# LIS-TU-Berlin/SVN-ICP

Hardware: AMD Instinct MI355X
Metric: scan-pair registrations/sec at N particles x M source pts, 1/2/4/8 GPU (higher is better)
Workload: dtype f64; 1 GPU; C3: 128 particles SVN-ICP, 131072-pt source vs 262144-pt target, K=100, I=20, max_dist=1.0, lr=1.0, SVNFullGrad=False, correspondence=fast, early stop off; synthetic 64-beam scans (seed 20250718); particles=128, target_points=262144, knn_count=100, parallelism=single GPU

## Files before the change

svn-icp_amd/csrc/api.hip:

```cpp
#include "../../include/svnicp_hip.h"

#include <cmath>
#include <algorithm>
#include <cstdio>
#include <cstdlib>
#include <cstring>
#include <string>
#include <vector>

#include "device_buffer.hpp"
#include "information_solve.hpp"
#include "kernels.hpp"
#include "stage_a_host.hpp"
#include "stage_b_host.hpp"

using namespace svnicp;
using namespace svnicp_host;

namespace {

struct CloudState {
  DevBuf<double> src, tgt;
  bool src_set = false, tgt_set = false;
};

struct SteinState {
  DevBuf<double> init_pose, R, t, Rtot, pose_out, eul, opt, uctl, work, stats;
  DevBuf<float> history;
  DevBuf<int> ctl;
  int hist_I = 0, hist_P = 0;
  PinnedBuf<double> h_init, h_stats;
  bool host_stats_valid = false;
  Event ev_init;
  bool init_in_flight = false;
  StepPlan step;
  DrivePlan drive;
  int single_done_it = -1;
  Event ev_fork, ev_join;
  bool median_pending = false;
  DevBuf<unsigned int> small_bar;
  bool small_launched = false;
  Event ev_chunk[3];
  PinnedBuf<int> h_flags;
  bool finish_seen = true;
  int finish_iter = 0;
};

struct Sharding {
  int p_lo = 0, p_hi = 0;
  bool set = false;
  int row_rank = 0, row_world = 1;
  int64_t B_total = 0;
  DevBuf<double> rank_sums;
};

struct MiniBatch {
  int batch = 0;
  uint64_t seed = 0, n = 0;
  bool explicit_tab = false;
  int tab_I = 0;
  std::vector<int32_t> tab_h;
  int64_t tab_checked_B = -1;
// ... 349 lines not shown
  if (!name || !value) return fail(c, SVNICP_ERR_INVALID, "svnicp_set_option: null argument");
  const std::string k(name), v(value);
  Tuning& t = c->tune;
  auto num = [&](int lo, int hi, int* out) { char* end = nullptr; const long x = strtol(v.c_str(), &end, 10);
                                             if (end == v.c_str() || *end || x < lo || x > hi) return false; *out = (int)x; return true; };
  bool ok = true;
  if (k == "knn") { if (v == "auto") t.knn = {}; else if (v == "v1") t.knn = {false, KnnKernel::Stream}; else if (v == "v2") t.knn = {false, KnnKernel::SeededScan};
                    else if (v == "brute") t.knn = {false, KnnKernel::Brute}; else if (v == "tiles") t.knn = {false, KnnKernel::Tiles}; else ok = false; }
  else if (k == "knn_prefilter") { if (v == "mfma") t.knn_prefilter_mfma = 1; else if (v == "valu") t.knn_prefilter_mfma = 0; else ok = false; }
  else if (k == "fallback_sliced_max") ok = num(-1, 1 << 20, &t.fallback_sliced_max);
  else if (k == "accum") { if (v == "f64") t.accum = 0; else if (v == "valu") t.accum = 1; else if (v == "split") t.accum = 3; else ok = false; }
  else if (k == "update") { if (v == "auto") t.update_fused = 0; else if (v == "fused") t.update_fused = 1; else ok = false; }
  else if (k == "fused_update_max_p") ok = num(1, 700, &t.fused_update_max_p);
  else if (k == "wgpcu") { int x = 0, y = 0; ok = sscanf(v.c_str(), "%d,%d", &x, &y) == 2 && x >= 0 && x <= 64 && y >= 0 && y <= 16; if (ok) { t.wgpcu_search = x; t.wgpcu_accum = y; } }
  else if (k == "tp") ok = num(0, 1 << 16, &t.tp);
  else if (k == "debug") ok = num(0, 1, &t.debug);
  else if (k == "scan_split") ok = num(0, 16, &t.scan_split);
  else if (k == "group_stride") ok = num(0, 1 << 30, &t.group_stride);
  else if (k == "accum_min_steps") ok = num(0, 1 << 20, &t.accum_min_steps);
  else if (k == "brute_qb") { ok = num(0, 6, &t.brute_qb); }
  else if (k == "single") { if (v == "fused") t.single_fused = 1; else if (v == "split") t.single_fused = 0; else ok = false; }
  else if (k == "chain") { if (v == "auto") { t.small_chain = 1; t.persistent = 0; } else if (v == "persistent") { t.small_chain = 1; t.persistent = 1; }
                           else if (v == "general") { t.small_chain = 0; t.persistent = 0; } else ok = false; }
  else if (k == "median") { if (v == "auto") t.median_inline = -1; else if (v == "stream") t.median_inline = 0; else if (v == "inline") t.median_inline = 1; else ok = false; }
  else if (k == "sort") { if (v == "joint") t.sort_joint = 1; else if (v == "separate") t.sort_joint = 0; else ok = false; }
  else if (k == "sort_kernel") { if (v == "radix") t.sort_merge = 0; else if (v == "merge") t.sort_merge = 1; else ok = false; }
  else if (k == "table") { if (v == "select") t.table_select = 1; else if (v == "gather") t.table_select = 0; else ok = false; }
  else if (k == "correspondence") { if (v == "fast") t.full_corr = 0; else if (v == "full") t.full_corr = 1; else ok = false; }
  else return fail(c, SVNICP_ERR_INVALID, "svnicp_set_option: unknown option '" + k + "'");
  if (!ok) return fail(c, SVNICP_ERR_INVALID, "svnicp_set_option: bad value '" + v + "' for option '" + k + "'");
  c->run.have_candidates = false;
  c->sa.held = TargetLayout::None;
  if (c->run.began) c->st.step = plan_step(registration_facts(c, c->pl.on), c->tune, c->sb.plan);
  return SVNICP_OK;
}

int svnicp_set_shard(svnicp_ctx* c, int p_lo, int p_hi) {
  CTX_CHECK(c);
  if (!c->run.particles_set || p_lo < 0 || p_hi > c->P || p_lo > p_hi)
    return fail(c, SVNICP_ERR_INVALID, "svnicp_set_shard: need 0 <= p_lo <= p_hi <= P after svnicp_set_particles");
  c->shard.p_lo = p_lo; c->shard.p_hi = p_hi; c->shard.set = true;
  return SVNICP_OK;
}

int svnicp_set_row_shard(svnicp_ctx* c, int row_rank, int row_world, int64_t total_source_points) {
  CTX_CHECK(c);
  if (!c->run.particles_set || row_world < 1 || row_rank < 0 || row_rank >= row_world || (row_world > 1 && total_source_points < 1))
// ... 53 lines not shown
  if (r.mb) {
    HIPCHK(c, c->mb.idx.ensure((size_t)r.Bt)); HIPCHK(c, c->mb.flag.ensure((size_t)B)); HIPCHK(c, c->mb.pos.ensure((size_t)B));
    HIPCHK(c, c->mb.bsum.ensure((size_t)minibatch_scan_blocks(B))); HIPCHK(c, c->mb.ctl.ensure(2));
    HIPCHK(c, c->mb.src_u.ensure((size_t)r.Bq * 3)); HIPCHK(c, c->mb.src.ensure((size_t)r.Bt * 3));
    HIPCHK(c, c->mb.cand.ensure((size_t)r.Bt * c->K));
  }
  if (const int rc = c->sb.begin(c, f, c->tune, r, shape, c->num_cus)) return rc;
  HIPCHK(c, c->st.history.ensure((size_t)(I > 0 ? I : 1) * 6 * P));
  c->st.hist_I = I; c->st.hist_P = P;
  if (c->prm.record_trace) {
    const size_t IP = (size_t)I * P;
    HIPCHK(c, c->tr.corr.ensure(IP * r.Bi));
    HIPCHK(c, hipMemsetAsync(c->tr.corr.p, 0xff, IP * r.Bi * 4, c->stream));
    const struct { DevBuf<double>& buf; size_t n; } dbl[] = {{c->tr.H, IP * 36}, {c->tr.b, IP * 6}, {c->tr.N, IP * 6}, {c->tr.phi, IP * 6}, {c->tr.h, (size_t)I + 1}};
    for (const auto& x : dbl) {
      HIPCHK(c, x.buf.ensure(x.n));
      HIPCHK(c, hipMemsetAsync(x.buf.p, 0, x.n * 8, c->stream));
    }
  }
  c->prof.pused = 0;
  c->st.single_done_it = -1;
  if (c->st.median_pending) HIPCHK(c, hipStreamWaitEvent(c->stream, c->st.ev_join, 0));
  c->st.median_pending = false;
  if (!c->st.finish_seen && c->prm.mode == SVNICP_MODE_SVGD && c->prm.check_early_stop) {
    int v[2] = {0, 0};
    HIPCHK(c, hipMemcpyAsync(v, c->st.ctl.p, sizeof v, hipMemcpyDeviceToHost, c->stream));
    HIPCHK(c, hipStreamSynchronize(c->stream));
    if (v[0]) c->st.finish_iter = v[1];
    c->st.finish_seen = true;
  }
  {
    BeginZero z{};
    auto add = [&](void* p, size_t bytes) { if (p && bytes) { z.ptr[z.n] = static_cast<unsigned int*>(p); z.dwords[z.n] = (unsigned int)(bytes / 4); ++z.n; } };
    add(c->st.uctl.p, update_uctl_doubles(P) * sizeof(double));
    add(c->st.history.p, (size_t)(I > 0 ? I : 1) * 6 * P * sizeof(float));
    add(c->sb.ambig.p, 2 * sizeof(int));
    if (c->sa.plan.kernel == KnnKernel::Brute) add(c->sa.fail_count.p, sizeof(int));
    HIPCHK(c, c->st.small_bar.ensure(8));
    add(c->st.small_bar.p, 8 * sizeof(unsigned int));
    if (c->prm.mode == SVNICP_MODE_SVGD) add(c->st.opt.p, (size_t)P * 18 * sizeof(double));
    const bool sa_words = c->sa.layout_pending;
    if (sa_words) {
      add(c->sa.bbox.p + 3, 3 * sizeof(unsigned long long)); add(c->sa.emax.p, sizeof(unsigned long long)); add(c->sa.fail_count.p, sizeof(int));
      z.ones = reinterpret_cast<unsigned int*>(c->sa.bbox.p); z.ones_dwords = 6;
    }
    z.ctl = c->st.ctl.p; z.iterations = I;
// ... 170 lines not shown
  c->st.median_pending = true;
  return SVNICP_OK;
}

int svnicp_iter_accumulate(svnicp_ctx* c, int it) {
  CTX_CHECK(c);
  if (!c->run.began || !c->run.have_candidates)
    return fail(c, SVNICP_ERR_INVALID, "svnicp_iter_accumulate: candidates not staged");
  if (it < 0 || it >= c->prm.iterations) return fail(c, SVNICP_ERR_INVALID, "svnicp_iter_accumulate: bad iteration");
  if (bind(c)) return SVNICP_ERR_HIP;
  if (const int rc = fork_median(c, it)) return rc;
  const int nshard = c->shard.p_hi - c->shard.p_lo;
  if (nshard <= 0) return SVNICP_OK;
  AccumArgs a = accum_args(c, it);
  if (c->tune.full_corr) {
    HIPCHK(c, prof_begin(c, KC_SEARCH));
    for (int p = c->shard.p_lo; p < c->shard.p_hi; ++p) {
      HIPCHK(c, launch_transform_cloud(c->cloud.src.p, c->B, c->st.Rtot.p + 12 * (size_t)p, c->sb.full_q.p, c->st.ctl.p, c->stream));
      if (const int rc = c->sa.search_blocks(c, stage_a_env(c), c->sb.full_q.p, c->B, 1, c->sb.full_idx.p + (size_t)p * c->B, c->sb.full_d2.p, 1)) return rc;
    }
    HIPCHK(c, prof_end(c));
    a.full_idx = c->sb.full_idx.p;
  } else if (c->sb.plan.f32 == 3) {
    HIPCHK(c, prof_begin(c, KC_SEARCH));
    HIPCHK(c, launch_search_split(c->sb.plan, a, c->stream));
    HIPCHK(c, prof_end(c));
  }
  if (c->pl.on) {
    PlaneArgs pa{};
    pa.src = c->cloud.src.p; pa.rec = c->pl.rec.p; pa.Rtot = c->st.Rtot.p; pa.B = c->B; pa.M = c->M; pa.p_lo = c->shard.p_lo; pa.p_hi = c->shard.p_hi;
    pa.max_dist = c->prm.max_dist; pa.delta = c->pl.delta; pa.partial = c->pl.partial.p; pa.ctl = c->st.ctl.p;
    pa.kidx = c->sb.kidx.p; pa.kbest = c->sb.kbest.p; pa.corr = a.corr;
    HIPCHK(c, prof_begin(c, KC_ACCUM));
    HIPCHK(c, launch_plane_accumulate(c->sb.plan, pa, c->stream));
    HIPCHK(c, prof_end(c));
    HIPCHK(c, prof_begin(c, KC_REDUCE));
    HIPCHK(c, launch_plane_finalize(c->pl.partial.p, c->sb.plan.grid_x, c->sb.plan.Ppad, c->shard.p_lo, nshard, c->pl.Hb.p, c->pl.stats.p,
                                    c->st.ctl.p, c->stream));
    HIPCHK(c, prof_end(c));
    return SVNICP_OK;
  }
  const bool single = c->st.step.single_fused;
  const UpdateArgs us = update_args(c, it);
  HIPCHK(c, prof_begin(c, KC_ACCUM));
  HIPCHK(c, launch_accumulate(c->sb.plan, a, single ? &us : nullptr, c->stream));
  HIPCHK(c, prof_end(c));
  if (single) { c->st.single_done_it = it; return SVNICP_OK; }
  if (c->st.step.chain == StepChain::SmallChain) return SVNICP_OK;
  HIPCHK(c, prof_begin(c, KC_REDUCE));
// ... 8 lines not shown
  if (!c->run.began) return fail(c, SVNICP_ERR_INVALID, "svnicp_iter_update: call svnicp_align_begin first");
  if (it < 0 || it >= c->prm.iterations) return fail(c, SVNICP_ERR_INVALID, "svnicp_iter_update: bad iteration");
  if (bind(c)) return SVNICP_ERR_HIP;
  if (c->st.single_done_it == it) { c->st.single_done_it = -1; return SVNICP_OK; }
  if (const int rc = ensure_dbg_upd(c)) return rc;
  UpdateArgs u = update_args(c, it);
  HIPCHK(c, prof_begin(c, KC_UPDATE));
  if (c->tune.debug && it == c->prm.iterations - 1)
    if (const int rc = print_update_phases(c, false)) return rc;
  const StepChain chain = c->st.step.chain;
  if (chain == StepChain::OneKernel) {
    u.svgd = 0;
    if (c->prm.mode == SVNICP_MODE_SVGD) HIPCHK(c, launch_update_svgd(u, c->stream));
    else HIPCHK(c, launch_update(u, c->stream));
  } else {
    if (chain == StepChain::SmallChain) {
      u.sums = c->sb.partial.p; u.n_ranks = c->sb.plan.grid_x; u.sums_stride = c->sb.plan.Ppad * kNSums; u.sums_out = c->sb.sums.p;
    }
    if (chain == StepChain::SideStream) {
      if (const int rc = fork_median(c, it)) return rc;
      HIPCHK(c, launch_update_prepare(u, c->stream));
      HIPCHK(c, hipStreamWaitEvent(c->stream, c->st.ev_join, 0));
      c->st.median_pending = false;
    } else {
      HIPCHK(c, launch_update_prepare_median(u, c->stream));
    }
    HIPCHK(c, launch_update_direction(u, c->stream, step_finishes(c, it)));
  }
  HIPCHK(c, prof_end(c));
  return SVNICP_OK;
}

static int enqueue_scoring(svnicp_ctx* c, double gate) {
  const bool normals = c->pl.supplied || c->pl.estimated;
  if (score_tile_rows(c->P, c->K, normals) < 1)
    return fail(c, SVNICP_ERR_INVALID, std::string(kScoringRefusal) + "knn_count is too large for one row's candidates to fit the scoring kernel's LDS tile");
  ScoreState& sc = c->sc;
  sc.have = false;
  HIPCHK(c, sc.partial.ensure((size_t)score_blocks(c->B) * score_padded_particles(c->P, c->K) * kScoreRecord));
  HIPCHK(c, sc.scores.ensure((size_t)c->P * kScoreFields));
  HIPCHK(c, sc.poses.ensure((size_t)c->P * 12));
  ScoreArgs a{};
  a.src = c->cloud.src.p; a.tgt = c->cloud.tgt.p; a.rec = normals ? c->pl.rec.p : nullptr; a.cand = c->sa.cand_idx.p; a.Rtot = c->st.Rtot.p;
  a.B = c->B; a.M = c->M; a.K = c->K; a.P = c->P; a.thr2 = gate * gate; a.partial = sc.partial.p;
  HIPCHK(c, launch_particle_score(a, sc.scores.p, c->stream));
  HIPCHK(c, hipMemcpyAsync(sc.poses.p, c->st.Rtot.p, (size_t)c->P * 12 * sizeof(double), hipMemcpyDeviceToDevice, c->stream));
// ... 656 lines not shown
```

svn-icp_amd/csrc/kernels.hpp:

```cpp
#pragma once
#include "device_math.hpp"
#include "registration_plan.hpp"
#include "stage_a_plan.hpp"

namespace svnicp {

struct KnnArgs {
  const double* src;
  Pose0 pose;
  const double *tx, *ty, *tz;
  const int32_t* torig;
  int64_t M, Mp;
  int64_t b_lo, b_hi;
  int K, S;
  double* pool_d;
  int32_t* pool_i;
  int32_t* out_idx;
  double* out_d2;
  const int32_t* qlist;
  const int* qlist_count;
  int list_grid;
  int list_qw;
  int slices, slice_max_queries, merge_n;
  double* sl_d;
// ... 106 lines not shown
  int tiles_per_block;
  int64_t n_tiles;
  int Ppad;
  double max_dist;
  double* partial;
  const int* ctl;
  int32_t* corr;
  int svgd;
  const double* tgt;
  const int32_t* cand;
  const double* anchor;
  int64_t M;
  uint8_t* kbest;
  int32_t* kidx;
  const int32_t* full_idx;
  int pts_per_block, spts_per_block;
  unsigned int* ticket;
  int fin_iteration, fin_P;
  double fin_thr;
  const double* fin_norms;
  const double* fin_pose;
  float* fin_history;
  int* fin_ctl;
};
AccumPlan plan_accumulate(AccumPlan shape, int64_t B, int num_cus, const Tuning& tune);
hipError_t launch_search_split(const AccumPlan& plan, AccumArgs a, hipStream_t st);
hipError_t launch_accumulate_split(const AccumPlan& plan, const AccumArgs& a, hipStream_t st);
void split_occupancy_blocks(int PW, int WP, int K, size_t smem, int* search, int* accum);
hipError_t launch_build_table3(const int32_t* idx, int64_t B, int K, const double* tgt, int64_t M, double* table,
                               double* anchor, float4* tablea, float* cmax, hipStream_t st);
hipError_t launch_build_table3_list(const int32_t* idx, const int32_t* list, const int* count, int64_t B, int K, const double* tgt,
                                    int64_t M, double* anchor, float4* tablea, float* cmax, hipStream_t st);
hipError_t launch_build_table2(const int32_t* idx, int64_t B, int K, const double* tgt, int64_t M, double* table,
                               float4* tablef, float* cmax, hipStream_t st);
hipError_t launch_transform_cloud(const double* src, int64_t B, const double* pose12, double* q, const int* ctl, hipStream_t st);
struct UpdateArgs {
  const double* sums;
  int n_ranks;
  int sums_stride;
  double* sums_out;
  double* R;
  double* t;
  double* Rtot;
  Pose0 pose;
  int P, iteration, iterations;
  double lr, conv_thr;
// ... 152 lines not shown
```

svn-icp_amd/csrc/registration_plan.hpp:

```cpp
#pragma once
#include <cstddef>
#include <cstdint>
#include <initializer_list>

#include "stage_a_plan.hpp"

namespace svnicp {

struct Tuning {
  KnnOption knn;
  int knn_prefilter_mfma = 1;
  int fallback_sliced_max = -1;
  int accum = 3;
  int update_fused = 0;
  int fused_update_max_p = 128;
  int wgpcu_search = 0, wgpcu_accum = 0;
  int tp = 0;
  int accum_min_steps = 0;
  int group_stride = 0;
  int scan_split = 0;
  int debug = 0;
  int single_fused = 1;
  int small_chain = 1;
  int persistent = 0;
// ... 142 lines not shown
  AccumPlan pl = stage_b_shape(stage_b_variant(t.accum, f.K, f.nshard(), t.full_corr != 0, f.plane), f.nshard(), f.K);
  pl.small = small_registration(pl, f, t, Bi) ? 1 : 0;
  return pl;
}

inline bool select_writes_table(const RegistrationFacts& f, const Tuning& t, const StageAPlan& a, const AccumPlan& b) {
  return t.table_select && a.kernel == KnnKernel::Tiles && a.K == f.K && b.f32 == 3 && f.batch == 0 && !f.shard_set;
}

inline bool joint_morton_sort(const RegistrationFacts& f, const Tuning& t, const StageAPlan& a) {
  return t.sort_joint && a.kernel == KnnKernel::Tiles && a.rows == f.B && f.batch == 0 && !f.shard_set;
}

enum class StepChain {
  OneKernel,
  SmallChain,
  InlineMedian,
  SideStream,
};
constexpr int kMedianInlineMaxP = 128;

struct StepPlan {
  StepChain chain = StepChain::OneKernel;
  bool single_fused = false;
};
inline StepPlan plan_step(const RegistrationFacts& f, const Tuning& t, const AccumPlan& pl) {
  StepPlan s;
  if (f.P < 2 || (t.update_fused && f.P <= t.fused_update_max_p)) s.chain = StepChain::OneKernel;
  else if (pl.small) s.chain = StepChain::SmallChain;
  else if (f.P <= kMedianInlineMaxP && f.P <= t.fused_update_max_p && t.median_inline != 0) s.chain = StepChain::InlineMedian;
  else s.chain = StepChain::SideStream;
  s.single_fused = f.P == 1 && !f.svgd && f.row_world == 1 && f.p_lo == 0 && f.p_hi == 1 && !t.full_corr && t.single_fused && pl.f32 == 1 &&
                   !f.plane;
  return s;
}

inline bool small_registration_supported(int PW, int WP, int K) {
  return K >= 97 && K <= 100 && ((WP == 1 && (PW == 16 || PW == 32 || PW == 64)) || (PW == 64 && WP == 2));
}

constexpr int kChunk = 4;
struct DrivePlan {
  bool persistent_try = false;
  bool defer_fin = false;
  bool follow = false;
};
inline DrivePlan plan_drive(const RegistrationFacts& f, const Tuning& t, const AccumPlan& pl, const StepPlan& s, bool blocking) {
  DrivePlan d;
  d.persistent_try = s.chain == StepChain::SmallChain && t.persistent && !f.record_trace && !f.profiling && f.I > 0 &&
                     small_registration_supported(pl.PW, pl.WP, f.K);
  d.defer_fin = f.check_early_stop && !f.record_trace && pl.f32 == 3 && !t.full_corr && s.chain != StepChain::OneKernel;
  d.follow = blocking && f.check_early_stop && f.I > 2 * kChunk;
  return d;
}
// ... 3 lines not shown
```

svn-icp_amd/csrc/stein_split.hip:

```cpp
#include "stein_split_device.hpp"

namespace svnicp {

namespace {

__device__ __forceinline__ void build_table3_row(const int32_t* __restrict__ idx, int64_t b, int K, const double* __restrict__ tgt, int64_t M,
                                                 double* __restrict__ table, double* __restrict__ anchor, float4* __restrict__ tablea,
                                                 float* __restrict__ cmax, float* rb, int lane) {
  int64_t i0 = idx[b * K];
  i0 = i0 < 0 ? 0 : (i0 >= M ? M - 1 : i0);
  const double a0 = tgt[3 * i0], a1 = tgt[3 * i0 + 1], a2 = tgt[3 * i0 + 2];
  float cm = 0.0f;
  for (int k = lane; k < 128; k += kWave) {
    float4 row = table_sentinel_row();
    if (k < K) {
      int64_t i = idx[b * K + k];
      i = i < 0 ? 0 : (i >= M ? M - 1 : i);
      const double x = tgt[3 * i], y = tgt[3 * i + 1], z = tgt[3 * i + 2];
      if (table) {
        double* o = table + ((size_t)b * K + k) * 3;
        o[0] = x; o[1] = y; o[2] = z;
      }
      row = table_row(x, y, z, a0, a1, a2);
      cm = table_row_cmax(cm, row);
// ... 21 lines not shown
}

constexpr int kTableListGrid = 64;
__global__ __launch_bounds__(256) void k_build_table3_list(const int32_t* __restrict__ idx, const int32_t* __restrict__ list,
                                                           const int* __restrict__ count, int64_t B, int K,
                                                           const double* __restrict__ tgt, int64_t M, double* __restrict__ anchor,
                                                           float4* __restrict__ tablea, float* __restrict__ cmax) {
  __shared__ __align__(16) float rowbuf[4][128 * 4];
  const int lane = threadIdx.x & (kWave - 1), wave = threadIdx.x >> 6;
  const int64_t n = *count;
  for (int64_t e = (int64_t)blockIdx.x * 4 + wave; e < n && e < B; e += (int64_t)gridDim.x * 4) {
    const int64_t b = list[e];
    if (b < 0 || b >= B) continue;
    build_table3_row(idx, b, K, tgt, M, nullptr, anchor, tablea, cmax, rowbuf[wave], lane);
    __builtin_amdgcn_wave_barrier();
  }
}


inline int row_code_for(int K) { return K <= 16 ? 1 : K <= 32 ? 2 : K <= 64 ? 4 : K <= 96 ? 6 : K <= 100 ? 60 : K <= 112 ? 7 : 8; }

template <int PW, int WP, int NRB, bool TAIL>
hipError_t launch_s(const AccumPlan& plan, const AccumArgs& a, hipStream_t st) {
  hipLaunchKernelGGL((k_stein_search_bf16<PW, WP, NRB, TAIL>), dim3(plan.sgrid_x, plan.grid_y), dim3(NT), 0, st, a);
  return hipGetLastError();
}
template <int PW, int WP>
hipError_t launch_srb(const AccumPlan& plan, const AccumArgs& a, hipStream_t st) {
  switch (row_code_for(a.K)) {
    case 1: return launch_s<PW, WP, 1, false>(plan, a, st);
    case 2: return launch_s<PW, WP, 2, false>(plan, a, st);
    case 4: return launch_s<PW, WP, 4, false>(plan, a, st);
    case 6: return launch_s<PW, WP, 6, false>(plan, a, st);
    case 60: return launch_s<PW, WP, 6, true>(plan, a, st);
    case 7: return launch_s<PW, WP, 7, false>(plan, a, st);
    default: return launch_s<PW, WP, 8, false>(plan, a, st);
  }
}
template <int PW, int WP>
hipError_t launch_w(const AccumPlan& plan, const AccumArgs& a, hipStream_t st) {
  if (!a.svgd && !a.corr && !a.full_idx) hipLaunchKernelGGL((k_stein_accumulate_w<PW, WP, true>), dim3(plan.grid_x, plan.grid_y), dim3(NT), plan.smem, st, a);
  else if (a.svgd && !a.corr && !a.full_idx) hipLaunchKernelGGL((k_stein_accumulate_w<PW, WP, true, true>), dim3(plan.grid_x, plan.grid_y), dim3(NT), plan.smem, st, a);
  else hipLaunchKernelGGL((k_stein_accumulate_w<PW, WP, false>), dim3(plan.grid_x, plan.grid_y), dim3(NT), plan.smem, st, a);
  return hipGetLastError();
}

template <int PW, int WP, int NRB, bool TAIL>
// ... 24 lines not shown
void split_occupancy_blocks(int PW, int WP, int K, size_t smem, int* search, int* accum) {
  return dispatch_lanes(PW, WP, [&](auto l) { return occ_split<l.PW, l.WP>(K, smem, search, accum); });
}

hipError_t launch_build_table3(const int32_t* idx, int64_t B, int K, const double* tgt, int64_t M, double* table,
                               double* anchor, float4* tablea, float* cmax, hipStream_t st) {
  if (B <= 0) return hipSuccess;
  hipLaunchKernelGGL(k_build_table3, dim3((unsigned)((B + 3) / 4)), dim3(256), 0, st, idx, B, K, tgt, M, table, anchor, tablea,
                     cmax);
  return hipGetLastError();
}

hipError_t launch_build_table3_list(const int32_t* idx, const int32_t* list, const int* count, int64_t B, int K, const double* tgt,
                                    int64_t M, double* anchor, float4* tablea, float* cmax, hipStream_t st) {
  if (B <= 0) return hipSuccess;
  hipLaunchKernelGGL(k_build_table3_list, dim3(kTableListGrid), dim3(256), 0, st, idx, list, count, B, K, tgt, M, anchor, tablea, cmax);
  return hipGetLastError();
}


hipError_t launch_search_split(const AccumPlan& plan, AccumArgs a, hipStream_t st) {
  a.Ppad = plan.Ppad; a.pts_per_block = plan.pts_per_block; a.spts_per_block = plan.spts_per_block;
  if (!search_offsets_fit(a.Ppad, a.K)) return hipErrorInvalidValue;
  return dispatch_lanes(plan.PW, plan.WP, [&](auto l) { return launch_srb<l.PW, l.WP>(plan, a, st); });
}

__global__ __launch_bounds__(256) void k_transform_cloud(const double* __restrict__ src, int64_t B, const double* __restrict__ pose12,
                                                         double* __restrict__ q, const int* __restrict__ ctl) {
  if (ctl[0]) return;
  const int64_t b = (int64_t)blockIdx.x * blockDim.x + threadIdx.x;
  if (b >= B) return;
  const double s0 = src[3 * b], s1 = src[3 * b + 1], s2 = src[3 * b + 2];
  q[3 * b] = (s0 * pose12[0] + s1 * pose12[1] + s2 * pose12[2]) + pose12[9];
  q[3 * b + 1] = (s0 * pose12[3] + s1 * pose12[4] + s2 * pose12[5]) + pose12[10];
  q[3 * b + 2] = (s0 * pose12[6] + s1 * pose12[7] + s2 * pose12[8]) + pose12[11];
}

hipError_t launch_transform_cloud(const double* src, int64_t B, const double* pose12, double* q, const int* ctl, hipStream_t st) {
  if (B <= 0) return hipSuccess;
  hipLaunchKernelGGL(k_transform_cloud, dim3((unsigned)((B + 255) / 256)), dim3(256), 0, st, src, B, pose12, q, ctl);
  return hipGetLastError();
}

hipError_t launch_accumulate_split(const AccumPlan& plan, const AccumArgs& a, hipStream_t st) {
  return dispatch_lanes(plan.PW, plan.WP, [&](auto l) { return launch_w<l.PW, l.WP>(plan, a, st); });
}
// ... 3 lines not shown
```

svn-icp_amd/csrc/stein_split_device.hpp:

```cpp
#pragma once
#include <cstdlib>
#include "kernels.hpp"
#include "stein_common.hpp"
#include "lane_fold_device.hpp"
#include "search_limits.hpp"

namespace svnicp {

namespace {

typedef float v4f __attribute__((ext_vector_type(4)));
#define SVNICP_CONST_AS __attribute__((address_space(4)))

__device__ __forceinline__ float pack_slot(float v, unsigned int mask, unsigned int bits) {
  return __uint_as_float((__float_as_uint(v) & ~mask) | bits);
}
__device__ __forceinline__ float imin_f(float a, float b) {
  const int x = (int)__float_as_uint(a), y = (int)__float_as_uint(b);
  return __uint_as_float((unsigned int)(x < y ? x : y));
}
__device__ __forceinline__ float imax_f(float a, float b) {
  const int x = (int)__float_as_uint(a), y = (int)__float_as_uint(b);
  return __uint_as_float((unsigned int)(x > y ? x : y));
}

constexpr float kSentinelCC = 1.0e30f;
__device__ __forceinline__ float4 table_row(double x, double y, double z, double a0, double a1, double a2) {
  const float cx = (float)(x - a0), cy = (float)(y - a1), cz = (float)(z - a2);
// ... 93 lines not shown
    const double d = (dx * dx + dy * dy) + dz * dz;
    if (k == 0) d_first = d;
    if (k < K && (d < bd || (d == bd && k < bk))) { bd = d; bk = k; }
  }
#pragma unroll
  for (int off = G / 2; off > 0; off >>= 1) {
    const double od = __shfl_xor(bd, off, kWave);
    const int ok = __shfl_xor(bk, off, kWave);
    if (od < bd || (od == bd && ok < bk)) { bd = od; bk = ok; }
  }
  const double d0 = __shfl(d_first, (threadIdx.x & (kWave - 1)) & ~(G - 1), kWave);
  return (d0 != d0 || bk == 0x7fffffff) ? 0 : bk;
}

#ifndef SVNICP_SEARCH_EPS_U
#define SVNICP_SEARCH_EPS_U 54
#endif
constexpr float kEpsBf16 = (float)SVNICP_SEARCH_EPS_U * 5.9604644775390625e-08f;

#ifndef SVNICP_SEARCH_WAVES
#define SVNICP_SEARCH_WAVES 4
#endif
template <int PW, int WP, int NRB, bool TAIL>
__device__ __forceinline__ void search_body(const AccumArgs& a, int bx, int by) {
  if (a.ctl[0]) return;
  if (a.fin_iteration >= 0 && bx == 0 && by == 0) {
    __shared__ double sh_fin[NT];
    __shared__ int sh_fin_stop;
    const int ftid = threadIdx.x, FP = a.fin_P;
    double fs = 0.0;
    for (int p = ftid; p < FP; p += NT) fs += a.fin_norms[p];
    sh_fin[ftid] = fs;
    __syncthreads();
    for (int off = NT / 2; off > 0; off >>= 1) {
      if (ftid < off) sh_fin[ftid] += sh_fin[ftid + off];
      __syncthreads();
    }
    if (ftid == 0) {
      const double m = sh_fin[0] / FP;
      const int stop = (float)m < (float)a.fin_thr;
      if (stop) { a.fin_ctl[0] = 1; a.fin_ctl[1] = a.fin_iteration + 1; }
      sh_fin_stop = stop;
    }
    __syncthreads();
    if (sh_fin_stop) return;
    for (int e = ftid; e < 6 * FP; e += NT) a.fin_history[(size_t)a.fin_iteration * 6 * FP + e] = (float)a.fin_pose[e];
  }
  constexpr int BW = kWave / PW;
  constexpr int CBP = PW / 16;
  constexpr int NPT = 4 / CBP;
  constexpr int ST = 4 * BW;
  constexpr bool PIPE = NPT == 1;
  constexpr int NTILE = 4 * NRB + (TAIL ? 1 : 0);
  constexpr int RS = 16 * (((4 * NTILE + 15) / 16) | 1);
  __shared__ float4 s_rows[4][NPT][4][RS / 4];
  __shared__ float4 s_scr4[4][64];
  __shared__ double s_pose[WP][12][64];
  __shared__ unsigned int s_queue[kQueueCap];
  __shared__ unsigned int s_qn, s_qsteps;
  const int tid = threadIdx.x;
  if (tid == 0) { s_qn = 0u; s_qsteps = 0u; }
#pragma unroll
  for (int i = 0; i < kQueueCap / NT; ++i) s_queue[tid + i * NT] = 0xffffffffu;
  const int lane = tid & (kWave - 1);
  const int wave = __builtin_amdgcn_readfirstlane(tid >> 6);
  const int pl = lane % PW, bs = lane / PW;
  const int mj = lane & 15, mk = lane >> 4;
  const int pbase = by * (WP * PW);
  for (int g = wave; g < WP; g += 4) {
    const int p = a.p_lo + pbase + g * PW + pl;
    const double* rp = a.Rtot + 12 * (size_t)(p < a.p_hi ? p : a.p_lo);
#pragma unroll
    for (int i = 0; i < 12; ++i) s_pose[g][i][lane] = rp[i];
  }
  const int K = a.K;
  const SVNICP_CONST_AS v4f* ctab = (const SVNICP_CONST_AS v4f*)a.tablea;
  float* const rows_w = reinterpret_cast<float*>(&s_rows[wave][0][mk][0]) + mj;
  const int64_t blk_lo = (int64_t)bx * a.spts_per_block;
  const int64_t blk_hi = (blk_lo + a.spts_per_block < a.B) ? blk_lo + a.spts_per_block : a.B;
  static_assert(BW <= kSearchPointsPerStep, "search_limits.hpp bounds the pair offsets for at most this many points per step");
  __syncthreads();
  const int64_t nfirst = blk_lo + wave * BW;
// ... 238 lines not shown

  if (pend_have) *(int32_t*)((char*)pend_row + pend_off4) = pend_idx;
  __syncthreads();
  {
    const unsigned int total = s_qn < (unsigned int)kQueueCap ? s_qn : (unsigned int)kQueueCap;
    constexpr int kExactLanes = 32;
    const int sub = lane & (kExactLanes - 1);
    for (unsigned int e = (unsigned int)(tid / kExactLanes); e < total; e += NT / kExactLanes) {
      const unsigned int ent = s_queue[e];
      if (ent == 0xffffffffu) continue;
      const int64_t be = blk_lo + (int64_t)(ent >> 8);
      const int pin = (int)(ent & 0xffu);
      const int ke = exact_nearest_of_k<kExactLanes>(a, s_pose[pin / PW], be, pin % PW, K, sub);
      if (sub == 0) {
        a.kbest[(size_t)be * a.Ppad + (pbase + pin)] = (uint8_t)ke;
        a.kidx[(size_t)be * a.Ppad + (pbase + pin)] = a.cand[(size_t)be * K + ke];
      }
    }
    if (tid == 0 && a.ambig_count && s_qsteps) { atomicAdd(a.ambig_count, (int)s_qsteps); atomicAdd(a.ambig_count + 1, (int)s_qn); }
  }
}

template <int PW, int WP, int NRB, bool TAIL>
__global__ __launch_bounds__(NT, (PW == 16 || WP == 4) ? 3 : SVNICP_SEARCH_WAVES) void k_stein_search_bf16(AccumArgs a) {
  search_body<PW, WP, NRB, TAIL>(a, xcd_block((int)blockIdx.x, (int)gridDim.x), (int)blockIdx.y);
}

template <int PW, int WP, bool PLAIN, bool SVGD = false>
__device__ __forceinline__ void accumulate_body(const AccumArgs& a, int bx, int by, double* lds) {
  if (a.ctl[0]) return;
#ifndef SVNICP_ACCUM_U
#define SVNICP_ACCUM_U 4
#endif
  constexpr int U = SVNICP_ACCUM_U;
  using Lanes = ParticleLanes<PW, WP>;
  constexpr int BW = Lanes::BW, STEP = Lanes::STEP;
  const Lanes L(by);
  const int wb = L.wb, bs = L.bs, pidx = L.pidx;
  const int p = a.p_lo + pidx;
  const bool pvalid = p < a.p_hi;

  double Rt[9], tt[3];
  load_pose(a.Rtot + 12 * (size_t)(pvalid ? p : a.p_lo), Rt, tt);
  double acc[kNSums];
#pragma unroll
  for (int i = 0; i < kNSums; ++i) acc[i] = 0.0;
  const int K = a.K;
  const int64_t blk_lo = (int64_t)bx * a.pts_per_block;
// ... 129 lines not shown
```

svn-icp_amd/csrc/stein_step_device.hpp:

```cpp
#pragma once
#include "kernels.hpp"

namespace svnicp {
namespace {

constexpr int UT = 512;
constexpr int KREG = 32;

struct PhaseStamp {
  unsigned long long* dbg;
  unsigned long long t;
  __device__ PhaseStamp(unsigned long long* d, bool mine) : dbg(mine ? d : nullptr), t(d ? __builtin_readcyclecounter() : 0ull) {}
  __device__ __forceinline__ void operator()(int i) {
    if (!dbg) return;
    const unsigned long long now = __builtin_readcyclecounter();
    dbg[i] += now - t;
    t = now;
  }
};

__device__ inline void finalize_Hb(const double* s, const double* Rc, double* H, double* b) {
  const double sw = s[0];
  const double a0 = s[1], a1 = s[2], a2 = s[3];
  const double xx = s[4], xy = s[5], xz = s[6], yy = s[7], yz = s[8], zz = s[9];
// ... 190 lines not shown
      unsigned int incl = tot;
#pragma unroll
      for (int off = 1; off < kWave; off <<= 1) {
        const unsigned int v = __shfl_up(incl, off, kWave);
        if (lane >= off) incl += v;
      }
      unsigned int cum = incl - tot;
      const unsigned int rank = S->rank;
#pragma unroll
      for (int i = 0; i < 4; ++i) {
        if (rank >= cum && rank < cum + c[i]) {
          S->prefix = (pre << 8) | (unsigned long long)(4 * lane + i);
          S->rank = rank - cum;
        }
        cum += c[i];
      }
    }
    __syncthreads();
  }
  return S->prefix;
}

template <int T>
__device__ __attribute__((noinline)) void rbf_bandwidth(const double* lx, int P, double* sq_global, SelShared* S, int tid, int lane, int wave) {
  const int n = P * P;
  const bool keys_in_regs = n <= KREG * T;
  const float invP = 1.0f / (float)P;
  unsigned long long key[KREG];
  if (keys_in_regs) {
#pragma unroll
    for (int i = 0; i < KREG; ++i) {
      const int e = i * T + tid;
      key[i] = ~0ull;
      if (e < n) {
        int r = (int)((float)e * invP);
        if (r * P > e) --r;
        if ((r + 1) * P <= e) ++r;
        const double s = pair_sq(lx, r, e - r * P);
        key[i] = (unsigned long long)__double_as_longlong(s);
        if (s != s) S->nan_flag = 1;
      }
    }
  } else {
    for (int e = tid; e < n; e += T) {
      const int r = e / P;
      const double s = pair_sq(lx, r, e - r * P);
      sq_global[e] = s;
      if (s != s) S->nan_flag = 1;
    }
    __syncthreads();
  }
  const int nk = (n - tid + T - 1) / T;
  block_select([&](auto count) {
    if (keys_in_regs) {
#pragma unroll
      for (int i = 0; i < KREG; ++i)
        if (i < nk) count(key[i]);
    } else {
      for (int e = tid; e < n; e += T) count((unsigned long long)__double_as_longlong(sq_global[e]));
    }
  }, 7, S, lane, wave);
  if (tid == 0) {
    const double med = S->nan_flag ? __builtin_nan("") : __longlong_as_double((long long)S->prefix);
    S->h = med / log((double)(P + 1));
  }
  __syncthreads();
}

constexpr int UCTL_H = 2, UCTL_HINV = 3, UCTL_NAN = 40, UCTL_BIN = 42, UCTL_RANK = 43, UCTL_CNT = 44,
              UCTL_NORM = 64;
constexpr int HB_OCT = 48, HB_NB = HB_OCT * 256, HB_EXP0 = 1023 - 40;
constexpr int SEL_LDS_KEYS = 16384;
constexpr int COLL_CHUNK = 4096;

__device__ __forceinline__ int key_bin(unsigned long long k) {
  const long long kb = (long long)(k >> 44) - ((long long)HB_EXP0 << 8);
  return kb < 0 ? 0 : (kb >= HB_NB ? HB_NB - 1 : (int)kb);
}
__device__ __forceinline__ unsigned int* upd_hist(double* uctl, int P) {
  return reinterpret_cast<unsigned int*>(uctl + UCTL_NORM + ((P + 7) & ~7));
}

__device__ void svgd_gradient(const UpdateArgs& a, int p, double* g6);
__device__ double svgd_step_one(const UpdateArgs& a, int p, const double* phi6, const double* xold6);

constexpr int PREP_T = 256, PREP_CH = 128, PREP_PW = 64;
struct PrepShared { double H[PREP_CH][37]; double Hmean[36]; };

__device__ __forceinline__ void prepare_body(const UpdateArgs& a, int bx) {
  if (a.ctl[0]) return;
  __shared__ PrepShared sh;
  const int tid = threadIdx.x, P = a.P;
  Work w(a.work, P);
  const int n_pw = (P + PREP_PW - 1) / PREP_PW;
  if (bx < n_pw) {
    const int p = bx * PREP_PW + tid;
    if (tid >= PREP_PW || p >= P) return;
    if (a.svgd) {
      double g6[6];
      svgd_gradient(a, p, g6);
// ... 10 lines not shown
    for (int i = 0; i < 6; ++i) { w.b[p * 6 + i] = b[i]; w.N[p * 6 + i] = N[i]; }
    return;
  }
  double hsum = 0.0;
  for (int c0 = 0; c0 < P; c0 += PREP_CH) {
    const int p = c0 + tid;
    if (tid < PREP_CH && p < P) {
      double H[36], b[6];
      particle_Hb(a, p, H, b);
#pragma unroll
      for (int i = 0; i < 36; ++i) sh.H[tid][i] = H[i];
    }
    __syncthreads();
    const int cnt = P - c0 < PREP_CH ? P - c0 : PREP_CH;
    if (tid < 36)
      for (int q = 0; q < cnt; ++q) hsum += sh.H[q][tid];
    __syncthreads();
  }
  if (tid < 36) sh.Hmean[tid] = hsum / P;
  __syncthreads();
  if (tid < 6) inverse_column(sh.Hmean, tid, a.uctl + UCTL_HINV);
}

template <int T, class Hit>
__device__ __forceinline__ void bin_of_rank(const unsigned int* hist, unsigned int rank, unsigned int* wave_tot, Hit hit) {
  constexpr int CH = HB_NB / T;
  const int tid = threadIdx.x, lane = tid & (kWave - 1), wave = tid >> 6;
  unsigned int c[CH], tot = 0;
#pragma unroll
  for (int i = 0; i < CH; ++i) { c[i] = hist[tid * CH + i]; tot += c[i]; }
  unsigned int incl = tot;
#pragma unroll
  for (int off = 1; off < kWave; off <<= 1) {
    const unsigned int v = __shfl_up(incl, off, kWave);
    if (lane >= off) incl += v;
  }
  if (lane == kWave - 1) wave_tot[wave] = incl;
  __syncthreads();
  unsigned int cum = incl - tot;
  for (int wv = 0; wv < wave; ++wv) cum += wave_tot[wv];
#pragma unroll
  for (int i = 0; i < CH; ++i) {
    if (rank >= cum && rank < cum + c[i]) hit(tid * CH + i, rank - cum);
    cum += c[i];
  }
}

constexpr int FRONT_BUF = 2048;
template <int T>
__device__ __forceinline__ void median_body(const UpdateArgs& a) {
  if (a.ctl[0]) return;
  extern __shared__ __align__(16) double dyn[];
  const int tid = threadIdx.x, lane = tid & (kWave - 1), wave = tid >> 6;
  const int P = a.P;
  Work w(a.work, P);
  double* lx = dyn;
  double* lbuf = dyn + 6 * P;
  unsigned int* lh = reinterpret_cast<unsigned int*>(lbuf + FRONT_BUF + 8);
  __shared__ SelShared sel;
  __shared__ unsigned int sh_scan[T / kWave];
  __shared__ unsigned int sh_cnt;
  __shared__ int sh_bin, sh_rank, sh_nan;

  PhaseStamp stamp(a.dbg, tid == 0);
  for (int e = tid; e < HB_NB; e += T) lh[e] = 0u;
  if (tid == 0) { sh_cnt = 0u; sh_nan = 0; sh_bin = 0; sh_rank = 0; }
  for (int p = tid; p < P; p += T) {
#pragma unroll
    for (int d = 0; d < 6; ++d) { const double v = a.pose_out[d * P + p]; lx[p * 6 + d] = v; w.x[p * 6 + d] = v; }
  }
  __syncthreads();
  stamp(0);

  const int n = P * P;
  bool nan = false;
  constexpr int KH = ((KREG + 1) / 2 + 1) * (512 / T);
  const int Pe = P + (P & 1), W = Pe - 1, npair = (Pe / 2) * W;
  const int di = T / W, dj = T - di * W;
  double keys[KH];
  const int bin0 = key_bin(0ull);
  if (tid == 0) atomicAdd(&lh[bin0], (unsigned int)P);
  for (int p = tid; p < P; p += T) { const double sq = pair_sq(lx, p, p); if (sq != sq) nan = true; }
  {
    int ra = tid / W, c = tid - ra * W;
#pragma unroll
    for (int k = 0; k < KH; ++k) {
      const int e = tid + k * T;
      keys[k] = -1.0;
      const int i = c >= ra ? ra : Pe - 1 - ra, j = c >= ra ? c + 1 : Pe - 1 - c;
      if (e < npair && j < P) {
        const double sq = pair_sq(lx, i, j);
        if (sq != sq) nan = true;
        keys[k] = sq;
        atomicAdd(&lh[key_bin((unsigned long long)__double_as_longlong(sq))], 2u);
      }
      c += dj; ra += di;
      if (c >= W) { c -= W; ++ra; }
    }
  }
  if (nan) sh_nan = 1;
  __syncthreads();
  stamp(1);
  bin_of_rank<T>(lh, (unsigned int)((n - 1) / 2), sh_scan, [&](int bin, unsigned int inside) { sh_bin = bin; sh_rank = (int)inside; });
  __syncthreads();
  stamp(2);
  const int bstar = sh_bin;
#pragma unroll
  for (int k = 0; k < KH; ++k) {
    if (keys[k] >= 0.0 && key_bin((unsigned long long)__double_as_longlong(keys[k])) == bstar) {
      const unsigned int pos = atomicAdd(&sh_cnt, 1u);
      if (pos < FRONT_BUF) lbuf[pos] = keys[k];
    }
  }
  __syncthreads();
  stamp(3);
  const int m = (int)sh_cnt;
  double med;
  if (m <= FRONT_BUF) {
    const int r = sh_rank;
    const bool zin = bstar == bin0;
    for (int e = m + tid; e < ((m + 7) & ~7); e += T) lbuf[e] = __builtin_nan("");
    __syncthreads();
    for (int e = tid; e < m; e += T) {
      const double v = lbuf[e];
      int lt = 0, eq = 0;
      for (int j0 = 0; j0 < m; j0 += 8) {
        double u[8];
#pragma unroll
        for (int t = 0; t < 8; ++t) u[t] = lbuf[j0 + t];
#pragma unroll
        for (int t = 0; t < 8; ++t) { lt += u[t] < v ? 1 : 0; eq += u[t] == v ? 1 : 0; }
      }
      const int LT = 2 * lt + ((zin && 0.0 < v) ? P : 0), EQ = 2 * eq + ((zin && v == 0.0) ? P : 0);
      if (LT <= r && r < LT + EQ) sel.h = v;
    }
    if (zin && tid == 0) {
      int eq0 = 0;
      for (int j = 0; j < m; ++j) eq0 += lbuf[j] == 0.0 ? 1 : 0;
      if (r < 2 * eq0 + P) sel.h = 0.0;
    }
    __syncthreads();
    med = sel.h;
  } else {
    sel_init(&sel, lower_median_rank(P), 0ull, tid);
    __syncthreads();
    rbf_bandwidth<T>(lx, P, w.sq, &sel, tid, lane, wave);
    med = sel.h * log((double)(P + 1));
    __syncthreads();
  }
  stamp(4);
  if (tid == 0) a.uctl[UCTL_H] = (sh_nan ? __builtin_nan("") : med) / log((double)(P + 1));
}

__device__ __forceinline__ double rbf_pair(const double* xi, const double* xj, double h, double* df) {
  double sq = 0.0;
#pragma unroll
  for (int d = 0; d < 6; ++d) { df[d] = xi[d] - xj[d]; sq += df[d] * df[d]; }
  return exp(-sq / h);
}


__device__ __forceinline__ void stein_direction_default(const double* x, const double* N, const double* Hinv, int P, double h,
                                                        const double* xi, bool act, int part, int tpp, double* phi) {
  double g[6] = {0, 0, 0, 0, 0, 0}, kn[6] = {0, 0, 0, 0, 0, 0}, ks = 0.0;
  if (act)
    for (int j = part; j < P; j += tpp) {
      double df[6];
      const double k = rbf_pair(xi, x + j * 6, h, df);
#pragma unroll
      for (int d = 0; d < 6; ++d) {
        g[d] += df[d] * k;
        kn[d] += k * (-N[j * 6 + d]);
      }
      ks += k;
// ... 245 lines not shown
    }
    a.eul[i] = v;
    e6[d] = v;
    const double df = v - xold6[d];
    n2 += df * df;
  }
  double Rm[9], Rt[9], tt[3];
  euler_to_R(e6[3], e6[4], e6[5], Rm);
  mat3_mul(a.pose.R0, Rm, Rt);
  mat3_vec(a.pose.R0, e6, tt);
#pragma unroll
  for (int i = 0; i < 9; ++i) { a.R[9 * p + i] = Rm[i]; a.Rtot[12 * p + i] = Rt[i]; }
#pragma unroll
  for (int i = 0; i < 3; ++i) { a.t[3 * p + i] = e6[i]; a.Rtot[12 * p + 9 + i] = a.pose.t0[i] + tt[i]; }
#pragma unroll
  for (int d = 0; d < 6; ++d) a.pose_out[d * P + p] = e6[d];
  return sqrt(n2);
}

__host__ __device__ inline int prepare_blocks(const UpdateArgs& a) {
  return (a.P + PREP_PW - 1) / PREP_PW + ((!a.svgd && !a.full_grad) ? 1 : 0);
}
__host__ __device__ inline int direction_blocks(int P) { return (P + 3) / 4; }
inline size_t median_lds_bytes(int P) {
  return (size_t)P * 6 * sizeof(double) + (size_t)(FRONT_BUF + 8) * sizeof(double) + (size_t)HB_NB * sizeof(unsigned int);
}

}
}
```

Before: 150.0 registrations/s.

## Compute RBF bandwidth median in an extra block of the search kernel

```diff
diff --git a/svn-icp_amd/csrc/api.hip b/svn-icp_amd/csrc/api.hip
--- a/svn-icp_amd/csrc/api.hip
+++ b/svn-icp_amd/csrc/api.hip
@@ -38,6 +38,7 @@
   int single_done_it = -1;
   Event ev_fork, ev_join;
   bool median_pending = false;
+  int stats_done_it = -1;
   DevBuf<unsigned int> small_bar;
   bool small_launched = false;
   Event ev_chunk[3];
@@ -433,7 +434,7 @@
   else if (k == "single") { if (v == "fused") t.single_fused = 1; else if (v == "split") t.single_fused = 0; else ok = false; }
   else if (k == "chain") { if (v == "auto") { t.small_chain = 1; t.persistent = 0; } else if (v == "persistent") { t.small_chain = 1; t.persistent = 1; }
                            else if (v == "general") { t.small_chain = 0; t.persistent = 0; } else ok = false; }
-  else if (k == "median") { if (v == "auto") t.median_inline = -1; else if (v == "stream") t.median_inline = 0; else if (v == "inline") t.median_inline = 1; else ok = false; }
+  else if (k == "median") { if (v == "auto") t.median_inline = -1; else if (v == "stream") t.median_inline = 0; else if (v == "inline") t.median_inline = 1; else if (v == "search") t.median_inline = 2; else ok = false; }
   else if (k == "sort") { if (v == "joint") t.sort_joint = 1; else if (v == "separate") t.sort_joint = 0; else ok = false; }
   else if (k == "sort_kernel") { if (v == "radix") t.sort_merge = 0; else if (v == "merge") t.sort_merge = 1; else ok = false; }
   else if (k == "table") { if (v == "select") t.table_select = 1; else if (v == "gather") t.table_select = 0; else ok = false; }
@@ -533,6 +534,7 @@
   c->st.single_done_it = -1;
   if (c->st.median_pending) HIPCHK(c, hipStreamWaitEvent(c->stream, c->st.ev_join, 0));
   c->st.median_pending = false;
+  c->st.stats_done_it = -1;
   if (!c->st.finish_seen && c->prm.mode == SVNICP_MODE_SVGD && c->prm.check_early_stop) {
     int v[2] = {0, 0};
     HIPCHK(c, hipMemcpyAsync(v, c->st.ctl.p, sizeof v, hipMemcpyDeviceToHost, c->stream));
@@ -749,9 +751,16 @@
     HIPCHK(c, prof_end(c));
     a.full_idx = c->sb.full_idx.p;
   } else if (c->sb.plan.f32 == 3) {
+    const bool stats = c->st.step.stats_in_search;
+    if (stats) {
+      if (const int rc = ensure_dbg_upd(c)) return rc;
+      const UpdateArgs u = update_args(c, it);
+      a.stat_P = u.P; a.stat_pose = u.pose_out; a.stat_work = u.work; a.stat_uctl = u.uctl; a.stat_dbg = u.dbg;
+    }
     HIPCHK(c, prof_begin(c, KC_SEARCH));
     HIPCHK(c, launch_search_split(c->sb.plan, a, c->stream));
     HIPCHK(c, prof_end(c));
+    if (stats) c->st.stats_done_it = it;
   }
   if (c->pl.on) {
     PlaneArgs pa{};
@@ -806,6 +815,9 @@
       HIPCHK(c, launch_update_prepare(u, c->stream));
       HIPCHK(c, hipStreamWaitEvent(c->stream, c->st.ev_join, 0));
       c->st.median_pending = false;
+    } else if (c->st.stats_done_it == it) {
+      HIPCHK(c, launch_update_prepare(u, c->stream));
+      c->st.stats_done_it = -1;
     } else {
       HIPCHK(c, launch_update_prepare_median(u, c->stream));
     }
diff --git a/svn-icp_amd/csrc/kernels.hpp b/svn-icp_amd/csrc/kernels.hpp
--- a/svn-icp_amd/csrc/kernels.hpp
+++ b/svn-icp_amd/csrc/kernels.hpp
@@ -152,6 +152,11 @@
   const double* fin_pose;
   float* fin_history;
   int* fin_ctl;
+  int stat_P;
+  double* stat_pose;
+  double* stat_work;
+  double* stat_uctl;
+  unsigned long long* stat_dbg;
 };
 AccumPlan plan_accumulate(AccumPlan shape, int64_t B, int num_cus, const Tuning& tune);
 hipError_t launch_search_split(const AccumPlan& plan, AccumArgs a, hipStream_t st);
diff --git a/svn-icp_amd/csrc/registration_plan.hpp b/svn-icp_amd/csrc/registration_plan.hpp
--- a/svn-icp_amd/csrc/registration_plan.hpp
+++ b/svn-icp_amd/csrc/registration_plan.hpp
@@ -188,6 +188,7 @@
 
 struct StepPlan {
   StepChain chain = StepChain::OneKernel;
+  bool stats_in_search = false;
   bool single_fused = false;
 };
 inline StepPlan plan_step(const RegistrationFacts& f, const Tuning& t, const AccumPlan& pl) {
@@ -196,6 +197,9 @@
   else if (pl.small) s.chain = StepChain::SmallChain;
   else if (f.P <= kMedianInlineMaxP && f.P <= t.fused_update_max_p && t.median_inline != 0) s.chain = StepChain::InlineMedian;
   else s.chain = StepChain::SideStream;
+  const bool ride_asked = t.median_inline == 2 || (t.median_inline < 0 && s.chain == StepChain::InlineMedian);
+  s.stats_in_search = (s.chain == StepChain::SmallChain || s.chain == StepChain::InlineMedian) && pl.f32 == 3 && !t.full_corr && ride_asked &&
+                      f.nshard() > 0;
   s.single_fused = f.P == 1 && !f.svgd && f.row_world == 1 && f.p_lo == 0 && f.p_hi == 1 && !t.full_corr && t.single_fused && pl.f32 == 1 &&
                    !f.plane;
   return s;
diff --git a/svn-icp_amd/csrc/stein_split.hip b/svn-icp_amd/csrc/stein_split.hip
--- a/svn-icp_amd/csrc/stein_split.hip
+++ b/svn-icp_amd/csrc/stein_split.hip
@@ -67,7 +67,7 @@
 
 template <int PW, int WP, int NRB, bool TAIL>
 hipError_t launch_s(const AccumPlan& plan, const AccumArgs& a, hipStream_t st) {
-  hipLaunchKernelGGL((k_stein_search_bf16<PW, WP, NRB, TAIL>), dim3(plan.sgrid_x, plan.grid_y), dim3(NT), 0, st, a);
+  hipLaunchKernelGGL((k_stein_search_bf16<PW, WP, NRB, TAIL>), dim3(plan.sgrid_x + (a.stat_P > 0 ? 1 : 0), plan.grid_y), dim3(NT), 0, st, a);
   return hipGetLastError();
 }
 template <int PW, int WP>
@@ -138,6 +138,7 @@
 hipError_t launch_search_split(const AccumPlan& plan, AccumArgs a, hipStream_t st) {
   a.Ppad = plan.Ppad; a.pts_per_block = plan.pts_per_block; a.spts_per_block = plan.spts_per_block;
   if (!search_offsets_fit(a.Ppad, a.K)) return hipErrorInvalidValue;
+  if (a.stat_P != 0 && (a.stat_P < 2 || a.stat_P > kStatMaxP)) return hipErrorInvalidValue;
   return dispatch_lanes(plan.PW, plan.WP, [&](auto l) { return launch_srb<l.PW, l.WP>(plan, a, st); });
 }
 
diff --git a/svn-icp_amd/csrc/stein_split_device.hpp b/svn-icp_amd/csrc/stein_split_device.hpp
--- a/svn-icp_amd/csrc/stein_split_device.hpp
+++ b/svn-icp_amd/csrc/stein_split_device.hpp
@@ -4,6 +4,7 @@
 #include "stein_common.hpp"
 #include "lane_fold_device.hpp"
 #include "search_limits.hpp"
+#include "stein_step_device.hpp"
 
 namespace svnicp {
 
@@ -143,7 +144,19 @@
 #define SVNICP_SEARCH_WAVES 4
 #endif
 template <int PW, int WP, int NRB, bool TAIL>
-__device__ __forceinline__ void search_body(const AccumArgs& a, int bx, int by) {
+struct SearchLds {
+  static constexpr int NPT = 4 / (PW / 16);
+  static constexpr int NTILE = 4 * NRB + (TAIL ? 1 : 0);
+  static constexpr int RS = 16 * (((4 * NTILE + 15) / 16) | 1);
+  float4 rows[4][NPT][4][RS / 4];
+  float4 scr4[4][64];
+  double pose[WP][12][64];
+  unsigned int queue[kQueueCap];
+  unsigned int qn, qsteps;
+};
+
+template <int PW, int WP, int NRB, bool TAIL>
+__device__ __forceinline__ void search_body(const AccumArgs& a, int bx, int by, SearchLds<PW, WP, NRB, TAIL>& lds) {
   if (a.ctl[0]) return;
   if (a.fin_iteration >= 0 && bx == 0 && by == 0) {
     __shared__ double sh_fin[NT];
@@ -174,11 +187,12 @@
   constexpr bool PIPE = NPT == 1;
   constexpr int NTILE = 4 * NRB + (TAIL ? 1 : 0);
   constexpr int RS = 16 * (((4 * NTILE + 15) / 16) | 1);
-  __shared__ float4 s_rows[4][NPT][4][RS / 4];
-  __shared__ float4 s_scr4[4][64];
-  __shared__ double s_pose[WP][12][64];
-  __shared__ unsigned int s_queue[kQueueCap];
-  __shared__ unsigned int s_qn, s_qsteps;
+  static_assert(NPT == SearchLds<PW, WP, NRB, TAIL>::NPT && RS == SearchLds<PW, WP, NRB, TAIL>::RS, "SearchLds states the same geometry");
+  float4 (&s_rows)[4][NPT][4][RS / 4] = lds.rows;
+  float4 (&s_scr4)[4][64] = lds.scr4;
+  double (&s_pose)[WP][12][64] = lds.pose;
+  unsigned int (&s_queue)[kQueueCap] = lds.queue;
+  unsigned int &s_qn = lds.qn, &s_qsteps = lds.qsteps;
   const int tid = threadIdx.x;
   if (tid == 0) { s_qn = 0u; s_qsteps = 0u; }
 #pragma unroll
@@ -463,8 +477,41 @@
 }
 
 template <int PW, int WP, int NRB, bool TAIL>
+__device__ __forceinline__ void search_body(const AccumArgs& a, int bx, int by) {
+  __shared__ SearchLds<PW, WP, NRB, TAIL> lds;
+  search_body<PW, WP, NRB, TAIL>(a, bx, by, lds);
+}
+
+constexpr int kStatBins = 64, kStatFront = 1024, kStatMaxP = 128;
+constexpr size_t kStatLdsBytes = median_lds_bytes(kStatMaxP, kStatBins, kStatFront);
+static_assert(kStatLdsBytes == 26688, "x 6 144 + front buffer 8 256 + histogram 12 288 bytes at 128 particles");
+
+template <int PW, int WP, int NRB, bool TAIL>
+union SearchLaunchLds {
+  SearchLds<PW, WP, NRB, TAIL> search;
+  double stat[kStatLdsBytes / sizeof(double)];
+};
+constexpr size_t kSearchLdsBeside = NT * sizeof(double) + sizeof(SelShared) + 64;
+
+__device__ __forceinline__ void pair_stats_ride(const AccumArgs& a, double* lds) {
+  UpdateArgs u{};
+  u.P = a.stat_P; u.pose_out = a.stat_pose; u.work = a.stat_work; u.uctl = a.stat_uctl; u.dbg = a.stat_dbg;
+  u.ctl = const_cast<int*>(a.ctl);
+  median_body<NT, kStatBins, kStatFront, false>(u, lds);
+}
+
+template <int PW, int WP, int NRB, bool TAIL>
 __global__ __launch_bounds__(NT, (PW == 16 || WP == 4) ? 3 : SVNICP_SEARCH_WAVES) void k_stein_search_bf16(AccumArgs a) {
-  search_body<PW, WP, NRB, TAIL>(a, xcd_block((int)blockIdx.x, (int)gridDim.x), (int)blockIdx.y);
+  constexpr int kPerCu = (PW == 16 || WP == 4) ? 3 : SVNICP_SEARCH_WAVES;
+  static_assert(kPerCu * (sizeof(SearchLaunchLds<PW, WP, NRB, TAIL>) + kSearchLdsBeside) <= 160 * 1024,
+                "the workgroups of a CU share 160 KB of LDS: the statistics' bytes alias the search arrays, they do not add to them");
+  __shared__ SearchLaunchLds<PW, WP, NRB, TAIL> lds;
+  const int ride = a.stat_P > 0 ? 1 : 0;
+  if (ride && blockIdx.x == 0) {
+    if (blockIdx.y == 0) pair_stats_ride(a, lds.stat);
+    return;
+  }
+  search_body<PW, WP, NRB, TAIL>(a, xcd_block((int)blockIdx.x - ride, (int)gridDim.x - ride), (int)blockIdx.y, lds.search);
 }
 
 template <int PW, int WP, bool PLAIN, bool SVGD = false>
diff --git a/svn-icp_amd/csrc/stein_step_device.hpp b/svn-icp_amd/csrc/stein_step_device.hpp
--- a/svn-icp_amd/csrc/stein_step_device.hpp
+++ b/svn-icp_amd/csrc/stein_step_device.hpp
@@ -236,7 +236,7 @@
 }
 
 template <int T>
-__device__ __attribute__((noinline)) void rbf_bandwidth(const double* lx, int P, double* sq_global, SelShared* S, int tid, int lane, int wave) {
+__device__ __forceinline__ void rbf_bandwidth_inline(const double* lx, int P, double* sq_global, SelShared* S, int tid, int lane, int wave) {
   const int n = P * P;
   const bool keys_in_regs = n <= KREG * T;
   const float invP = 1.0f / (float)P;
@@ -280,6 +280,10 @@
   }
   __syncthreads();
 }
+template <int T>
+__device__ __attribute__((noinline)) void rbf_bandwidth(const double* lx, int P, double* sq_global, SelShared* S, int tid, int lane, int wave) {
+  rbf_bandwidth_inline<T>(lx, P, sq_global, S, tid, lane, wave);
+}
 
 constexpr int UCTL_H = 2, UCTL_HINV = 3, UCTL_NAN = 40, UCTL_BIN = 42, UCTL_RANK = 43, UCTL_CNT = 44,
               UCTL_NORM = 64;
@@ -287,9 +291,14 @@
 constexpr int SEL_LDS_KEYS = 16384;
 constexpr int COLL_CHUNK = 4096;
 
+constexpr int hb_bins(int BPO) { return HB_OCT * BPO; }
+constexpr int hb_log2(int BPO) { return BPO <= 1 ? 0 : 1 + hb_log2(BPO / 2); }
+template <int BPO = 256>
 __device__ __forceinline__ int key_bin(unsigned long long k) {
-  const long long kb = (long long)(k >> 44) - ((long long)HB_EXP0 << 8);
-  return kb < 0 ? 0 : (kb >= HB_NB ? HB_NB - 1 : (int)kb);
+  constexpr int LG = hb_log2(BPO), NB = hb_bins(BPO);
+  static_assert((1 << LG) == BPO && LG <= 8, "bins per octave: a power of two, at most 256");
+  const long long kb = (long long)(k >> (52 - LG)) - ((long long)HB_EXP0 << LG);
+  return kb < 0 ? 0 : (kb >= NB ? NB - 1 : (int)kb);
 }
 __device__ __forceinline__ unsigned int* upd_hist(double* uctl, int P) {
   return reinterpret_cast<unsigned int*>(uctl + UCTL_NORM + ((P + 7) & ~7));
@@ -346,9 +355,10 @@
   if (tid < 6) inverse_column(sh.Hmean, tid, a.uctl + UCTL_HINV);
 }
 
-template <int T, class Hit>
+template <int T, int NB = HB_NB, class Hit>
 __device__ __forceinline__ void bin_of_rank(const unsigned int* hist, unsigned int rank, unsigned int* wave_tot, Hit hit) {
-  constexpr int CH = HB_NB / T;
+  static_assert(NB % T == 0, "a whole chunk of bins per thread");
+  constexpr int CH = NB / T;
   const int tid = threadIdx.x, lane = tid & (kWave - 1), wave = tid >> 6;
   unsigned int c[CH], tot = 0;
 #pragma unroll
@@ -371,10 +381,13 @@
 }
 
 constexpr int FRONT_BUF = 2048;
-template <int T>
-__device__ __forceinline__ void median_body(const UpdateArgs& a) {
+constexpr size_t median_lds_bytes(int P, int bpo = 256, int front = FRONT_BUF) {
+  return (size_t)P * 6 * sizeof(double) + (size_t)(front + 8) * sizeof(double) + (size_t)hb_bins(bpo) * sizeof(unsigned int);
+}
+template <int T, int BPO, int FB, bool CALL = true>
+__device__ __forceinline__ void median_body(const UpdateArgs& a, double* dyn) {
   if (a.ctl[0]) return;
-  extern __shared__ __align__(16) double dyn[];
+  constexpr int HB_NB = hb_bins(BPO), FRONT_BUF = FB;
   const int tid = threadIdx.x, lane = tid & (kWave - 1), wave = tid >> 6;
   const int P = a.P;
   Work w(a.work, P);
@@ -402,7 +415,7 @@
   const int Pe = P + (P & 1), W = Pe - 1, npair = (Pe / 2) * W;
   const int di = T / W, dj = T - di * W;
   double keys[KH];
-  const int bin0 = key_bin(0ull);
+  const int bin0 = key_bin<BPO>(0ull);
   if (tid == 0) atomicAdd(&lh[bin0], (unsigned int)P);
   for (int p = tid; p < P; p += T) { const double sq = pair_sq(lx, p, p); if (sq != sq) nan = true; }
   {
@@ -416,7 +429,7 @@
         const double sq = pair_sq(lx, i, j);
         if (sq != sq) nan = true;
         keys[k] = sq;
-        atomicAdd(&lh[key_bin((unsigned long long)__double_as_longlong(sq))], 2u);
+        atomicAdd(&lh[key_bin<BPO>((unsigned long long)__double_as_longlong(sq))], 2u);
       }
       c += dj; ra += di;
       if (c >= W) { c -= W; ++ra; }
@@ -425,13 +438,13 @@
   if (nan) sh_nan = 1;
   __syncthreads();
   stamp(1);
-  bin_of_rank<T>(lh, (unsigned int)((n - 1) / 2), sh_scan, [&](int bin, unsigned int inside) { sh_bin = bin; sh_rank = (int)inside; });
+  bin_of_rank<T, HB_NB>(lh, (unsigned int)((n - 1) / 2), sh_scan, [&](int bin, unsigned int inside) { sh_bin = bin; sh_rank = (int)inside; });
   __syncthreads();
   stamp(2);
   const int bstar = sh_bin;
 #pragma unroll
   for (int k = 0; k < KH; ++k) {
-    if (keys[k] >= 0.0 && key_bin((unsigned long long)__double_as_longlong(keys[k])) == bstar) {
+    if (keys[k] >= 0.0 && key_bin<BPO>((unsigned long long)__double_as_longlong(keys[k])) == bstar) {
       const unsigned int pos = atomicAdd(&sh_cnt, 1u);
       if (pos < FRONT_BUF) lbuf[pos] = keys[k];
     }
@@ -468,12 +481,18 @@
   } else {
     sel_init(&sel, lower_median_rank(P), 0ull, tid);
     __syncthreads();
-    rbf_bandwidth<T>(lx, P, w.sq, &sel, tid, lane, wave);
+    if constexpr (CALL) rbf_bandwidth<T>(lx, P, w.sq, &sel, tid, lane, wave);
+    else rbf_bandwidth_inline<T>(lx, P, w.sq, &sel, tid, lane, wave);
     med = sel.h * log((double)(P + 1));
     __syncthreads();
   }
   stamp(4);
   if (tid == 0) a.uctl[UCTL_H] = (sh_nan ? __builtin_nan("") : med) / log((double)(P + 1));
+}
+template <int T>
+__device__ __forceinline__ void median_body(const UpdateArgs& a) {
+  extern __shared__ __align__(16) double dyn[];
+  median_body<T, 256, FRONT_BUF>(a, dyn);
 }
 
 __device__ __forceinline__ double rbf_pair(const double* xi, const double* xj, double h, double* df) {
@@ -765,9 +784,6 @@
   return (a.P + PREP_PW - 1) / PREP_PW + ((!a.svgd && !a.full_grad) ? 1 : 0);
 }
 __host__ __device__ inline int direction_blocks(int P) { return (P + 3) / 4; }
-inline size_t median_lds_bytes(int P) {
-  return (size_t)P * 6 * sizeof(double) + (size_t)(FRONT_BUF + 8) * sizeof(double) + (size_t)HB_NB * sizeof(unsigned int);
-}
-
-}
-}
+
+}
+}
```

After: 152.2 registrations/s, median of 4. 1.4% higher.
